# igashov/DiffLinker

Measured on AMD Instinct MI355X. Metric: molecules/sec (500-step sample_chain), higher is better.
Workload: dtype f32 (f16x3 split MFMA, fp32 accumulate)

## Files before the change

### difflinker_amd/csrc/egnn_fc.hip

```cpp
#include <hip/hip_runtime.h>
#include <stdint.h>
#include <stdlib.h>
#include <string.h>
#include <math.h>
#include <cmath>

#include <algorithm>
#include <atomic>
#include <vector>

#include "../../include/difflinker_hip.h"
#include "pack_layout.h"


namespace {

constexpr int LDH = 132;
constexpr int NMAX = 55;
constexpr int NQMAX = 2 * NMAX;
constexpr int THREADS = 512;
constexpr int NWAVES = THREADS / 64;
constexpr int GWAVES = 8;
constexpr int GTHREADS = 64 * GWAVES;
constexpr int L_A = 0;
// ... 1477 lines not shown
    lds_barrier();
    prof_event(pf, w, lane, 250);
    if (valid) {
#pragma unroll
        for (int ot = 0; ot < 8; ++ot) {
            *reinterpret_cast<float4*>(v.A + l * LDH + 16 * ot + 4 * kg) = Pout[ot];
            *reinterpret_cast<float4*>(v.B + l * LDH + 16 * ot + 4 * kg) = Qout[ot];
        }
    }
    }
    if (tid == 0) {
        if constexpr (POST) { v.fmax[FS_HS] = __float_as_uint(s_hn); v.misc[CX_PAR] = par ^ 1; }
        v.misc[CX_PASS] = pass_open;
    }
    if constexpr (TEAM) {
        prof_event(pf, w, lane, 110);
        lds_barrier();
        team_exchange_q<1>(v, nb, tid, scn, pass_open == 0, POST ? (par ^ 1) : par, pf);
    }
    prof_event(pf, w, lane, 11);
    dma_wait();
    lds_barrier();
}


template <int PREC, bool TEAM, bool ATT>
__device__ __forceinline__ void gcl_pass3(const Lds& v, Prof& pf) {
    {
    const PassCtx cx = pass_ctx(v);
    const int nb = cx.nb, N = cx.N, par = cx.par;
    const int8_t* emask = cx.em;
    const float* sc = cx.g + G_SCALE;
    const LaneIds q = lane_ids(v);
    const int tid = q.tid, w = q.w, lane = q.lane;
    prof_event(pf, w, lane, 12);
    if (tid == 0) { v.fmax[FM_H0 + (par ^ 1)] = 0u; v.fmax[FM_AGG] = 0u; }
    const float hmax = __uint_as_float(v.fmax[TEAM ? FM_HG : FM_H0 + par]);
    const float x2 = __uint_as_float(v.fmax[FM_X2]), x02 = __uint_as_float(v.fmax[FM_X02]);
    const float pqb = (cload(sc, SC_L1_W1A) + cload(sc, SC_L1_W1B)) * hmax + cload(sc, SC_B1);
    const float u1b = pqb + 4.0f * (x2 * cload(sc, GS_WRW) + x02 * cload(sc, GS_WDW));
    const float sa = scale_for(u1b);
    const float accs = sa * cload(sc, 5);
    if (tid == 0 && (beyond_f16_range(u1b) || beyond_f16_range(hmax) || beyond_f16_range(4.0f * x2) || beyond_f16_range(4.0f * x02)))
        atomicOr(&v.misc[1], NAN_RANGE | 3);
    if constexpr (ATT) pair_phase<false, PREC, true, TEAM>(v, nb, w, lane, emask, N, 0.0f, sa, inv_pow2(accs), sc, cload(sc, 8), pf);
    else pair_phase<false, PREC, false, TEAM>(v, nb, w, lane, emask, N, 0.0f, sa, inv_pow2(accs), sc, 0.0f, pf);
    prof_event(pf, w, lane, 13);
    }
    AggRegs ar;
    bool next_eq;
    {
        const PassCtx cx = pass_ctx(v);
        const int nown = TEAM ? ctx_i(v, TM_NOWN) : cx.nb;
        const LaneIds q = lane_ids(v);
        next_eq = cx.nx.equiv;
        lds_barrier();
        prof_event(pf, q.w, q.lane, 20);
        const float am = pair_reduce_gcl(v, nown, cx.nb, q.tid, ar, (cx.flags & 4) ? 1.0f / float(cx.N) : 1.0f);
        block_max(&v.fmax[FM_AGG], am, q.lane);
        prof_event(pf, q.w, q.lane, 21);
        lds_barrier();
        prof_event(pf, q.w, q.lane, 22);
    }
    if (next_eq) stream_phase<TEAM, true, true>(v, pf, &ar);
    else stream_phase<TEAM, true, false>(v, pf, &ar);
}

template <int PREC, bool TEAM>
__device__ __forceinline__ void equiv_pass3(const Lds& v, Prof& pf) {
    {
    const PassCtx cx = pass_ctx(v);
    const int nb = cx.nb, N = cx.N, par = cx.par;
    const int8_t* emask = cx.em;
    const float* sc = cx.g + E_SCALE;
    const float norm_constant = ctx_f(v, CX_NORMC);
    const LaneIds q = lane_ids(v);
    const int w = q.w, lane = q.lane;
    prof_event(pf, w, lane, 32);
    const float hmax = __uint_as_float(v.fmax[TEAM ? FM_HG : FM_H0 + par]);
    const float x2 = __uint_as_float(v.fmax[FM_X2]), x02 = __uint_as_float(v.fmax[FM_X02]);
    const float pqb = (cload(sc, SCE_L1_W5A) + cload(sc, SCE_L1_W5B)) * hmax + cload(sc, SCE_B5);
    const float u1b = pqb + 4.0f * (x2 * cload(sc, ES_WRW) + x02 * cload(sc, ES_WDW));
    const float sa = scale_for(u1b);
    const float accs = sa * cload(sc, 2);
    if (q.tid == 0 && (beyond_f16_range(u1b) || beyond_f16_range(hmax) || beyond_f16_range(4.0f * x2) || beyond_f16_range(4.0f * x02)))
        atomicOr(&v.misc[1], NAN_RANGE | 3);
    const float phi = cload(sc, ES_W7L1) * fmaf(cload(sc, ES_L1_W6), u1b, cload(sc, ES_B6));
    const bool proven = 2.0f * float(nb) * phi < 1e37f;
    if (!proven) {
        const bool widen = ctx_i(v, MS_FULL) == 0;
        __syncthreads();
        if (widen) {
            const int tid_ = q.tid;
            receivers_all(v, TEAM ? ctx_i(v, TM_NOWN) : nb, tid_);
            __syncthreads();
        }
    }
    pair_phase<true, PREC, false, TEAM>(v, nb, w, lane, emask, N, norm_constant, sa, inv_pow2(accs), sc,
                                        (cx.flags & 2) ? ctx_f(v, CX_CRANGE) : 0.0f, pf);
    prof_event(pf, w, lane, 33);
    }
    const PassCtx cx = pass_ctx(v);
    const int nb = cx.nb, N = cx.N;
    const int nown = TEAM ? ctx_i(v, TM_NOWN) : nb;
    const int S = TEAM ? ctx_i(v, TM_S) : 1, rank = TEAM ? ctx_i(v, TM_RANK) : 0;
    const bool more = cx.nx.base != nullptr;
    const LaneIds q = lane_ids(v);
    const int tid = q.tid, lane = q.lane;
    lds_barrier();
    const float xscale = (cx.flags & 4) ? 1.0f / float(N) : ((cx.flags & 2) ? ctx_f(v, CX_INVNORM) : 1.0f);
    pair_reduce_equiv<true>(v, nown, nb, tid, xscale);
    if (tid == 0) v.fmax[TEAM ? FM_XOWN : FM_X2] = 0u;
    lds_barrier();
    const float* aggx = v.A - L_A + L_AGGX3;
    float n2 = 0.0f;
    if (tid < nown) {
        const float lm = v.lm[tid];
        const int a = rank + tid * S;
        const bool moves = v.rpos[tid] >= 0;
#pragma unroll
        for (int k = 0; k < 3; ++k) {
            float xn = v.xs[4 * a + k];
            if (moves) {
                xn += aggx[4 * tid + k] * lm;
                v.xs[4 * a + k] = xn;
            }
            n2 = fmaf(xn, xn, n2);
        }
    }
    block_max(&v.fmax[TEAM ? FM_XOWN : FM_X2], n2, lane);
    prof_event(pf, q.w, lane, 34);
    lds_barrier();
    prof_event(pf, q.w, lane, 10);
    if (more) stream_phase<TEAM, false, false>(v, pf, nullptr);
}

template <bool TEAM>
__device__ __forceinline__ void head_phase(const Lds& v, bool v3);

template <int PREC, bool TEAM, bool ATT>
__device__ __forceinline__ void forward_molecule2(const Lds& v, Prof& pf) {
    const int tid = lane_ids(v).tid;
    const int nb = ctx_i(v, 0);
    const int nown = TEAM ? ctx_i(v, TM_NOWN) : nb;
    const int S = TEAM ? ctx_i(v, TM_S) : 1, rank = TEAM ? ctx_i(v, TM_RANK) : 0;
    const float* wp = ctx_p<const float>(v, CX_WP);
    float* hs = ctx_p<float>(v, CX_HS);
    const float tfeat = ctx_f(v, CX_TFEAT);
    const int nf = ctx_i(v, CX_NF), fin = ctx_i(v, CX_FIN);
    const int npass = ctx_i(v, CX_NPASS);
    const int w = __builtin_amdgcn_readfirstlane(tid >> 6);
    const int lane = tid & 63;
    const bool v3 = (PREC != 0) && !TEAM && nown > 32;
    if (tid == 0) { v.misc[CX_PASS] = v3 ? -1 : 0; v.misc[CX_PAR] = 0; v.misc[CX_V3] = v3 ? 1 : 0; }
    if (tid < 8) reinterpret_cast<int*>(v.A - L_A + L_PROG)[tid] = 0;
    if (!TEAM && tid < HID) (v.A - L_A + L_ZROW)[tid] = 0.0f;
    prof_event(pf, w, lane, 1);
    {
        if (tid < 8) v.fmax[tid] = 0u;
        __syncthreads();
    }
    const NextPass first = {wp + OFF_BLOCKS, false};
    if (!v3) stage_next(v, first, w, tid);
    if (tid < 4 * nown) {
        const int l = tid >> 2, k = tid & 3, a = rank + l * S;
        const float xv = (k < 3) ? v.z[l * DMAX + k] : 0.0f;
        v.xs[4 * a + k] = xv;
        v.x0[4 * a + k] = xv;
    }
    {
        float n2 = 0.0f;
        if (tid < nown) {
            const float x0 = v.z[tid * DMAX], x1 = v.z[tid * DMAX + 1], x2 = v.z[tid * DMAX + 2];
            n2 = x0 * x0 + x1 * x1 + x2 * x2;
        }
        const unsigned b = wave_max_u32(__float_as_uint(n2));
        if (lane == 0) {
            if (TEAM) lds_max_u32(&v.fmax[FM_XOWN], b);
            else { lds_max_u32(&v.fmax[FM_X2], b); lds_max_u32(&v.fmax[FM_X02], b); }
        }
    }
    {
        const int f = tid & (HID - 1);
        float wrow[FINP];
        const float4* wsrc = reinterpret_cast<const float4*>(wp + OFF_EMB_W + f * FINP);
#pragma unroll
        for (int q = 0; q < FINP / 4; ++q) {
            const float4 t4 = wsrc[q];
            wrow[4 * q] = t4.x; wrow[4 * q + 1] = t4.y; wrow[4 * q + 2] = t4.z; wrow[4 * q + 3] = t4.w;
        }
        const float be = wp[OFF_EMB_B + f];
        const float* ctxp = ctx_p<const float>(v, CX_CTXP);
        const int ct = ctx_i(v, CX_CT);
        const int nctx = fin - nf - ct;
        float hmax = 0.0f;
        for (int l = tid >> 7; l < nown; l += THREADS / HID) {
            const int pos = v.idx[rank + l * S];
            float acc = be;
#pragma unroll
            for (int k = 0; k < FINP; ++k) {
                float hin = 0.0f;
                if (k < nf) hin = v.z[l * DMAX + 3 + k];
                else if (k < nf + ct) hin = tfeat;
                else if (k < fin) hin = ctxp[pos * nctx + (k - nf - ct)];
                acc = fmaf(wrow[k], hin, acc);
            }
            if (v3) {
                hs[HS_HT + ((((l >> 4) * 8 + (f >> 4)) * 64 + 16 * ((f >> 2) & 3) + (l & 15)) * 4) + (f & 3)] = acc;
            } else {
            v.B[l * LDH + f] = acc;
            {
                const int r = l & 31;
                hs[HS_HT + ((((l >> 5) * 4 + (f >> 5)) * 4 + (r >> 3)) * 64 + (f & 31) + 32 * ((r >> 2) & 1)) * 4 + (r & 3)] = acc;
            }
            }
            hmax = fmaxf(hmax, fabsf(acc));
        }
        block_max(&v.fmax[FM_H0], hmax, lane);
    }
    __syncthreads();
    if (v3) {
        if constexpr (PREC != 0 && !TEAM) {
        if (tid == 0 && beyond_f16_range(__uint_as_float(v.fmax[FM_H0]))) atomicOr(&v.misc[1], NAN_RANGE | 3);
        prof_event(pf, w, lane, 2);
        stream_phase<TEAM, false, false>(v, pf, nullptr);
        const int sub = ctx_i(v, CX_SUB);
#pragma nounroll
        for (int p = 0; p < npass; p += sub + 1) {
#pragma nounroll
            for (int gi = 0; gi < sub; ++gi) gcl_pass3<PREC, TEAM, ATT>(v, pf);
            equiv_pass3<PREC, TEAM>(v, pf);
        }
        prof_event(pf, w, lane, 3);
        __syncthreads();
        head_phase<TEAM>(v, true);
        }
    } else {
    {
        const float s0 = (PREC != 0) ? scale_for(__uint_as_float(v.fmax[FM_H0])) : 1.0f;
        for (int e = tid; e < nown * 32; e += THREADS)
            put_quad<PREC>(v.C + (e >> 5) * LDH, 4 * (e & 31), *reinterpret_cast<const float4*>(v.B + (e >> 5) * LDH + 4 * (e & 31)), s0);
        if (PREC != 0 && tid == 0) {
            v.fmax[FS_HS] = __float_as_uint(s0);
            if (beyond_f16_range(__uint_as_float(v.fmax[FM_H0]))) atomicOr(&v.misc[1], NAN_RANGE | 3);
        }
    }
    __syncthreads();
    prof_event(pf, w, lane, 2);
    {
        PreW2 pw;
        load_pre2(pw, first, w, lane, nown);
        open_pass<PREC, TEAM>(v, nb, nown, first, hs, pf, pw, 0, 0);
    }
    const int sub = ctx_i(v, CX_SUB);
#pragma nounroll
    for (int p = 0; p < npass; p += sub + 1) {
#pragma nounroll
        for (int gi = 0; gi < sub; ++gi) gcl_pass2<PREC, TEAM, ATT>(v, pf);
        equiv_pass2<PREC, TEAM>(v, pf);
    }
    prof_event(pf, w, lane, 3);
    __syncthreads();
    head_phase<TEAM>(v, false);
    }
    prof_event(pf, w, lane, 4);
}

template <bool TEAM>
__device__ __forceinline__ void head_phase(const Lds& v, bool v3) {
    const int tid = lane_ids(v).tid;
    const int nb = ctx_i(v, 0), nf = ctx_i(v, CX_NF);
    const int nown = TEAM ? ctx_i(v, TM_NOWN) : nb;
    const int S = TEAM ? ctx_i(v, TM_S) : 1, rank = TEAM ? ctx_i(v, TM_RANK) : 0;
    const float* wp = ctx_p<const float>(v, CX_WP);
    const float* hs = ctx_p<const float>(v, CX_HS);
    float* eps = v.A;
    int nanbits = 0;
    for (int e = tid; e < nown * nf; e += THREADS) {
        const int a = e / nf, o = e - a * nf;
        const int r = a & 31;
        const float* wo = wp + OFF_OUT_W + o * HID;
        float acc = wp[OFF_OUT_B + o];
        if (v3) {
            const float* hp = hs + HS_HT + ((a >> 4) * 8 * 64 + (a & 15)) * 4;
#pragma unroll
            for (int ot = 0; ot < 8; ++ot)
#pragma unroll
                for (int kg = 0; kg < 4; ++kg) {
                    const float4 hv = *reinterpret_cast<const float4*>(hp + (ot * 64 + 16 * kg) * 4);
                    const float4 wv = *reinterpret_cast<const float4*>(wo + 16 * ot + 4 * kg);
                    acc = fmaf(hv.x, wv.x, acc); acc = fmaf(hv.y, wv.y, acc);
                    acc = fmaf(hv.z, wv.z, acc); acc = fmaf(hv.w, wv.w, acc);
                }
        } else {
        const float* hp = hs + HS_HO + ((a >> 5) * 4 * 16 + (r & 3) + 4 * (r >> 3)) * 64 + 32 * ((r >> 2) & 1);
#pragma unroll
        for (int nt4 = 0; nt4 < 4; ++nt4)
#pragma unroll 8
            for (int q = 0; q < 8; ++q) {
                const float4 hv = *reinterpret_cast<const float4*>(hp + nt4 * 16 * 64 + 4 * q);
                const float4 wv = *reinterpret_cast<const float4*>(wo + 32 * nt4 + 4 * q);
                acc = fmaf(hv.x, wv.x, acc); acc = fmaf(hv.y, wv.y, acc);
                acc = fmaf(hv.z, wv.z, acc); acc = fmaf(hv.w, wv.w, acc);
            }
        }
        (void)r;
        eps[a * DMAX + 3 + o] = acc;
        if (acc != acc) nanbits |= 2;
    }
    if (tid < 4 * nown && (tid & 3) < 3) {
        const int l = tid >> 2, a = rank + l * S;
        const float vel = v.xs[4 * a + (tid & 3)] - v.x0[4 * a + (tid & 3)];
        eps[l * DMAX + (tid & 3)] = vel;
        if (vel != vel) nanbits |= 1;
    }
    if (TEAM && tid == 0 && v.misc[TM_FAIL] != 0) nanbits |= 8;
    if (nanbits) atomicOr(&v.misc[1], nanbits);
    __syncthreads();
}

__device__ __forceinline__ void build_receivers(const Lds& v, int nown, int tid) {
    if (tid < 64) {
        const bool rec = tid < nown && v.lm[tid] != 0.0f;
        const unsigned long long bal = __ballot(rec);
        const int pos = __popcll(bal & ((1ull << tid) - 1ull));
        if (rec) v.rcv[pos] = tid;
        if (tid < NMAX + 1) v.rpos[tid] = rec ? pos : -1;
        if (tid == 0) { v.misc[MS_NRCV] = __popcll(bal); v.misc[MS_FULL] = (__popcll(bal) == nown) ? 1 : 0; }
    }
}

__device__ __forceinline__ int compact_atoms(const Lds& v, const int8_t* __restrict__ node_mask_b, int N, int tid) {
    if (tid < 64) {
        int count = 0;
        for (int base = 0; base < N; base += 64) {
            const int a = base + tid;
            const bool real = (a < N) && (node_mask_b[a] != 0);
            const unsigned long long bal = __ballot(real);
            const int pos = count + __popcll(bal & ((1ull << tid) - 1ull));
            if (real && pos < NQMAX) v.idx[pos] = a;
            count += __popcll(bal);
        }
        if (tid == 0) { v.misc[0] = count; v.misc[1] = 0; }
    }
    __syncthreads();
    return v.misc[0];
}

struct FwdArgs {
    const float* wpack;
    ModelDims md;
    int B, N;
    const float* xh;
    const float* t;
    int t_stride;
    const int8_t* node_mask;
    const float* linker_mask;
    const int8_t* edge_mask;
    const float* context;
    float* out;
    int* nan_flags;
    unsigned long long* prof;
    int team;
    int team_fault;
    char* team_rows;
    unsigned* team_flags;
    float* hsave;
};

struct TeamSlot {
    int slot, rank;
};
__device__ __forceinline__ TeamSlot team_slot(int k, int S) {
    const int group = k / (8 * S), within = k - group * 8 * S;
    TeamSlot t;
    t.slot = group * 8 + (within & 7);
    t.rank = within >> 3;
    return t;
// ... 563 lines not shown
        for (int k = 0; k < HID; ++k) r += fabs(double(w[size_t(f) * ld + col0 + k]) * scale);
        m = fmax(m, r);
    }
    return float(m * 1.0001);
}

float pack_sin_columns(float* dst, const float* w, int ld, double scale) {
    double m = 0.0;
    for (int f = 0; f < HID; ++f) {
        double r = 0.0;
        for (int k = 0; k < SIN_K; ++k) {
            const double v = double(w[size_t(f) * ld + 2 * HID + k]) * scale;
            dst[k * HID + f] = float(v);
            r += fabs(v);
        }
        m = fmax(m, r);
    }
    return float(m * 1.0001);
}

float vec_absmax(const float* v) {
    float m = 0.0f;
    for (int f = 0; f < HID; ++f) m = fmaxf(m, fabsf(v[f]));
    return m;
}

void pack_vec(float* dst, const float* src, int stride, double scale) {
    for (int f = 0; f < HID; ++f) dst[f] = float(double(src[size_t(f) * stride]) * scale);
}

struct Balance {
    int perm[HID];
    double fac[HID];
};
void balance_hidden(Balance& b, const double* proxy, int group, bool on) {
    for (int p = 0; p < HID; ++p) { b.perm[p] = p; b.fac[p] = 1.0; }
    if (!on) return;
    double key[HID];
    for (int f = 0; f < HID; ++f) key[f] = std::isfinite(proxy[f]) ? proxy[f] : 1.7e308;
    proxy = key;
    std::stable_sort(b.perm, b.perm + HID, [&](int x, int y) { return proxy[x] > proxy[y]; });
    const double top = proxy[b.perm[0]];
    if (!(top > 0.0) || !std::isfinite(top)) return;
    int real = 0;
    while (real < HID && proxy[b.perm[real]] > 0.0) ++real;
    if (real < HID) {
        const int groups = HID / group, per = (real + groups - 1) / groups;
        int sorted[HID];
        memcpy(sorted, b.perm, sizeof(sorted));
        int pad = real;
        for (int g = 0; g < groups; ++g)
            for (int q = 0; q < group; ++q) {
                const int j = g * per + q;
                b.perm[g * group + q] = (q < per && j < real) ? sorted[j] : sorted[pad++];
            }
    }
    for (int p0 = 0; p0 < HID; p0 += group) {
        const double m = proxy[b.perm[p0]];
        int n = 0;
        if (m > 0.0 && std::isfinite(m)) {
            int et, em;
            frexp(top, &et); frexp(m, &em);
            n = std::min(std::max(et - em, 0), 40);
        } else n = 40;
        for (int p = p0; p < p0 + group; ++p) b.fac[p] = ldexp(1.0, n);
    }
}
void permute_rows(std::vector<float>& wp, std::vector<float>& bp, const float* w, const float* bias, int ld, const Balance& b) {
    wp.resize(size_t(HID) * ld); bp.resize(HID);
    for (int p = 0; p < HID; ++p) {
        memcpy(&wp[size_t(p) * ld], w + size_t(b.perm[p]) * ld, size_t(ld) * sizeof(float));
        bp[p] = bias[b.perm[p]];
    }
}
void permute_cols(std::vector<float>& wp, const float* w, const Balance& b) {
    wp.resize(size_t(HID) * HID);
    for (int f = 0; f < HID; ++f)
        for (int p = 0; p < HID; ++p) wp[size_t(f) * HID + p] = float(double(w[size_t(f) * HID + b.perm[p]]) / b.fac[p]);
}
float row_l1_weighted(const float* w, int ld, int col0, int ncols, double scale, const Balance& b) {
    double m = 0.0;
    for (int p = 0; p < HID; ++p) {
        double r = 0.0;
        for (int k = 0; k < ncols; ++k) r += fabs(double(w[size_t(p) * ld + col0 + k]) * scale);
        m = fmax(m, r * b.fac[p]);
    }
    return float(m * 1.0001);
}
float vec_absmax_weighted(const float* v, const Balance& b) {
    double m = 0.0;
    for (int p = 0; p < HID; ++p) m = fmax(m, fabs(double(v[p])) * b.fac[p]);
    return float(m * 1.0001);
}

}

extern "C" {

int32_t dl_abi_version(void) { return DL_ABI_VERSION; }
#ifdef DL_PROFILE
int32_t dl_profile_max_events(void) { return PROF_MAX_EVENTS; }
#else
int32_t dl_profile_max_events(void) { return 0; }
#endif
void dl_set_profile_buffer(void* device_buf) { g_prof_buf = static_cast<unsigned long long*>(device_buf); }
int32_t dl_last_hip_error(void) { return g_last_hip; }
int32_t dl_max_atoms(void) { return NMAX; }
#ifdef DL_TEST_HOOKS
void dl_debug_team_fault(int32_t launches) { g_team_fault.store(launches < 0 ? 0 : launches); }
#endif

const char* dl_error_string(int32_t s) {
    switch (s) {
        case DL_OK: return "ok";
        case DL_ERR_BAD_ARG: return "bad argument";
        case DL_ERR_UNSUPPORTED: return "hyper-parameter not supported by the HIP path";
        case DL_ERR_TOO_MANY_ATOMS: return "molecule exceeds dl_max_atoms()";
        case DL_ERR_HIP: return "HIP runtime error";
        case DL_ERR_NO_DEVICE: return "no HIP device";
        case DL_ERR_ALLOC: return "allocation failed";
        default: return "unknown";
    }
}

static int32_t check_cfg(const dl_config* c) {
    if (!c) return DL_ERR_BAD_ARG;
    if (c->n_dims != 3 || c->hidden_nf != HID) return DL_ERR_UNSUPPORTED;
    if (c->inv_sublayers < 1 || c->inv_sublayers > MAX_SUBLAYERS) return DL_ERR_UNSUPPORTED;
    if ((c->condition_time | 1) != 1) return DL_ERR_BAD_ARG;
    if (c->in_node_nf < 1 || 3 + c->in_node_nf > DMAX || c->in_node_nf > 16) return DL_ERR_UNSUPPORTED;
    if (c->context_node_nf < 0 || c->context_node_nf > CTXMAX) return DL_ERR_UNSUPPORTED;
    if (c->in_node_nf + c->condition_time + c->context_node_nf > FINP) return DL_ERR_UNSUPPORTED;
    if (c->n_layers < 1 || c->n_layers > 64) return DL_ERR_UNSUPPORTED;
    if (!(c->normalization_factor > 0.0f)) return DL_ERR_BAD_ARG;
    if (c->precision != DL_PRECISION_FP32 && c->precision != DL_PRECISION_F16X3 && c->precision != DL_PRECISION_F16X2) return DL_ERR_UNSUPPORTED;
    if ((c->attention | 1) != 1 || (c->tanh | 1) != 1 || (c->aggregation_mean | 1) != 1) return DL_ERR_BAD_ARG;
    if ((c->sin_embedding | 1) != 1) return DL_ERR_BAD_ARG;
    if (c->tanh && !(c->coords_range > 0.0f)) return DL_ERR_BAD_ARG;
    return DL_OK;
}

int32_t dl_model_num_tensors(const dl_config* cfg) {
    if (!cfg) return DL_ERR_BAD_ARG;
    return 4 + cfg->n_layers * (cfg->inv_sublayers * (8 + (cfg->attention ? 2 : 0)) + 5);
}

int32_t dl_model_create(const dl_config* cfg, const float* const* w, int32_t n_tensors, dl_model** out) {
    int32_t st = check_cfg(cfg);
    if (st != DL_OK) return st;
    if (!w || !out || n_tensors != dl_model_num_tensors(cfg)) return DL_ERR_BAD_ARG;
    for (int i = 0; i < n_tensors; ++i)
        if (!w[i]) return DL_ERR_BAD_ARG;
    const int nf = cfg->in_node_nf, fin = nf + cfg->condition_time + cfg->context_node_nf, L = cfg->n_layers, SUB = cfg->inv_sublayers;
    const size_t total = size_t(OFF_BLOCKS) + size_t(L) * block_size(SUB);
    float* hp = static_cast<float*>(calloc(total, sizeof(float)));
    if (!hp) return DL_ERR_ALLOC;
    const bool f16 = cfg->precision != DL_PRECISION_FP32;
    auto image = [&](float* d, const float* ww, int ld, double sc) -> float {
        if (f16) return float(pack_lds_image_f16(d, ww, ld, sc));
        pack_lds_image(d, ww, ld, sc);
        return 1.0f;
    };
    auto image_t = [&](float* d, const float* ww, int ld, double sc) {
        if (f16) (void)pack_lds_image_f16_t(d, ww, ld, sc);
        else pack_lds_image_t(d, ww, ld, sc);
    };
    const double c = -1.4426950408889634;
    const double inv_norm = 1.0 / double(cfg->normalization_factor);
    int ti = 0;
    const float* ew = w[ti++]; const float* eb = w[ti++];
    const float* ow = w[ti++]; const float* ob = w[ti++];
    for (int f = 0; f < HID; ++f) {
        for (int k = 0; k < fin; ++k) hp[OFF_EMB_W + f * FINP + k] = ew[size_t(f) * fin + k];
        hp[OFF_EMB_B + f] = eb[f];
    }
    for (int o = 0; o < nf; ++o) {
        memcpy(hp + OFF_OUT_W + o * HID, ow + size_t(o) * HID, HID * sizeof(float));
        hp[OFF_OUT_B + o] = ob[o];
    }
    std::vector<float> w1p, b1p, w2p, w3p, b3p, w4p;
    std::vector<double> proxy(HID);
    for (int blk = 0; blk < L; ++blk) {
        float* base = hp + OFF_BLOCKS + size_t(blk) * block_size(SUB);
        for (int gi = 0; gi < SUB; ++gi) {
            float* g = base + gi * GCL_SIZE;
            const float* w1 = w[ti++]; const float* b1 = w[ti++];
            const float* w2 = w[ti++]; const float* b2 = w[ti++];
            const float* w3 = w[ti++]; const float* b3 = w[ti++];
            const float* w4 = w[ti++]; const float* b4 = w[ti++];
            const float* watt = nullptr; const float* batt = nullptr;
            if (cfg->attention) { watt = w[ti++]; batt = w[ti++]; }
            const int ld1 = 2 * HID + (cfg->sin_embedding ? SIN_K : 2);
            const int nattr = ld1 - 2 * HID;
            const double s3b = cfg->aggregation_mean ? 1.0 : inv_norm;
            Balance be, bt;
            for (int f = 0; f < HID; ++f) {
                double r = fabs(double(b1[f]));
                for (int k = 0; k < 2 * HID; ++k) r += fabs(double(w1[size_t(f) * ld1 + k]));
                for (int k = 0; k < nattr; ++k) r += (cfg->sin_embedding ? 1.0 : 32.0) * fabs(double(w1[size_t(f) * ld1 + 2 * HID + k]));
                proxy[f] = r;
            }
            balance_hidden(be, proxy.data(), 16, f16);
            for (int f = 0; f < HID; ++f) {
                double r = fabs(double(b3[f]) * c);
                for (int k = 0; k < HID; ++k) r += fabs(double(w3[size_t(f) * 2 * HID + k]) * c) + fabs(double(w3[size_t(f) * 2 * HID + HID + k]) * s3b);
                proxy[f] = r;
            }
            balance_hidden(bt, proxy.data(), 32, f16);
            permute_rows(w1p, b1p, w1, b1, ld1, be);
            permute_cols(w2p, w2, be);
            permute_rows(w3p, b3p, w3, b3, 2 * HID, bt);
            permute_cols(w4p, w4, bt);
            float* sc = g + G_SCALE;
            if (f16) {
                pack_unit_f16(g + G_W1A, w1p.data(), ld1, 0, c, sc + GS_SW_W1A);
                pack_unit_f16(g + G_W1B, w1p.data(), ld1, HID, c, sc + GS_SW_W1B);
                pack_unit_f16(g + G_W3A, w3p.data(), 2 * HID, 0, c, sc + GS_SW_W3A);
                pack_unit_f16(g + G_W3B, w3p.data(), 2 * HID, HID, s3b, sc + GS_SW_W3B);
                sc[4] = float(pack_unit_f16_uniform(g + G_W4, w4p.data(), HID, 0, 1.0 / c));
                {
                    std::vector<float> ua(UNIT), ub(UNIT);
                    pack_stream_f16(ua.data(), w3p.data(), 2 * HID, 0, c, true);
                    pack_stream_f16(ub.data(), w3p.data(), 2 * HID, HID, s3b, true);
                    for (int h2 = 0; h2 < 2; ++h2) {
                        memcpy(g + G_ST_POST + (2 * h2 + 0) * ST_CHUNK, ua.data() + h2 * ST_CHUNK, ST_CHUNK * sizeof(float));
                        memcpy(g + G_ST_POST + (2 * h2 + 1) * ST_CHUNK, ub.data() + h2 * ST_CHUNK, ST_CHUNK * sizeof(float));
                    }
                }
                pack_stream_f16(g + G_ST_POST + 2 * UNIT, w4p.data(), HID, 0, 1.0 / c, false);
                pack_stream_f16(g + G_ST_PRE, w1p.data(), ld1, 0, c, true);
                pack_stream_f16(g + G_ST_PRE + UNIT, w1p.data(), ld1, HID, c, true);
            } else {
                pack_unit(g + G_W1A, w1p.data(), ld1, 0, c); pack_unit(g + G_W1B, w1p.data(), ld1, HID, c);
                pack_unit(g + G_W3A, w3p.data(), 2 * HID, 0, c); pack_unit(g + G_W3B, w3p.data(), 2 * HID, HID, s3b);
                pack_unit(g + G_W4, w4p.data(), HID, 0, 1.0 / c);
                for (int k = 0; k < 16; ++k) sc[GS_SW_W1A + k] = 1.0f;
                sc[4] = 1.0f;
            }
            sc[5] = image(g + G_W2, w2p.data(), HID, 1.0);
            image_t(g + G_W2T, w2p.data(), HID, 1.0);
            for (int s_ = 0; s_ < 8; ++s_) sc[GS_NE + s_] = float(be.fac[16 * s_]);
            for (int nt = 0; nt < 4; ++nt) sc[GS_NT + nt] = float(bt.fac[32 * nt]);
            float* vv = g + G_VEC;
            pack_vec(vv + 0 * HID, b1p.data(), 1, c);
            if (!cfg->sin_embedding) {
                pack_vec(vv + 1 * HID, w1p.data() + 2 * HID, ld1, c);
                pack_vec(vv + 2 * HID, w1p.data() + 2 * HID + 1, ld1, c);
            } else {
                (void)pack_sin_columns(g + G_WG, w1p.data(), ld1, c);
                sc[20] = row_l1_weighted(w1p.data(), ld1, 2 * HID, SIN_K, c, be);
            }
            pack_vec(vv + 3 * HID, b2, 1, c);
            pack_vec(vv + 4 * HID, b3p.data(), 1, c);
            pack_vec(vv + 5 * HID, b4, 1, 1.0);
            if (watt) { pack_vec(vv + 6 * HID, watt, 1, 1.0 / c); sc[8] = batt[0]; }
            sc[6] = vec_absmax(vv + 1 * HID);
            sc[7] = vec_absmax(vv + 2 * HID);
            sc[GS_WRW] = vec_absmax_weighted(vv + 1 * HID, be);
            sc[GS_WDW] = vec_absmax_weighted(vv + 2 * HID, be);
            sc[12] = row_l1_weighted(w1p.data(), ld1, 0, HID, c, be); sc[13] = row_l1_weighted(w1p.data(), ld1, HID, HID, c, be);
            sc[14] = row_l1_weighted(w3p.data(), 2 * HID, 0, HID, c, bt); sc[15] = row_l1_weighted(w3p.data(), 2 * HID, HID, HID, s3b, bt);
            sc[16] = row_l1(w4p.data(), HID, 0, 1.0 / c);
            sc[17] = vec_absmax_weighted(vv + 0 * HID, be); sc[18] = vec_absmax_weighted(vv + 4 * HID, bt);
            sc[19] = vec_absmax(vv + 5 * HID) * 1.0001f;
        }
        float* e = base + SUB * GCL_SIZE;
        const float* w5 = w[ti++]; const float* b5 = w[ti++];
        const float* w6 = w[ti++]; const float* b6 = w[ti++];
        const float* w7 = w[ti++];
        const int ld5 = 2 * HID + (cfg->sin_embedding ? SIN_K : 2);
        Balance bc;
        for (int f = 0; f < HID; ++f) {
            double r = fabs(double(b5[f]));
            for (int k = 0; k < 2 * HID; ++k) r += fabs(double(w5[size_t(f) * ld5 + k]));
            for (int k = 0; k < ld5 - 2 * HID; ++k) r += (cfg->sin_embedding ? 1.0 : 32.0) * fabs(double(w5[size_t(f) * ld5 + 2 * HID + k]));
            proxy[f] = r;
        }
        balance_hidden(bc, proxy.data(), 16, f16);
        permute_rows(w1p, b1p, w5, b5, ld5, bc);
        permute_cols(w2p, w6, bc);
        float* sc = e + E_SCALE;
        if (f16) {
            pack_unit_f16(e + E_W5A, w1p.data(), ld5, 0, c, sc + ES_SW_W5A);
            pack_unit_f16(e + E_W5B, w1p.data(), ld5, HID, c, sc + ES_SW_W5B);
            pack_stream_f16(e + E_ST_PRE, w1p.data(), ld5, 0, c, true);
            pack_stream_f16(e + E_ST_PRE + UNIT, w1p.data(), ld5, HID, c, true);
        } else {
            pack_unit(e + E_W5A, w1p.data(), ld5, 0, c); pack_unit(e + E_W5B, w1p.data(), ld5, HID, c);
            for (int k = 0; k < 8; ++k) sc[ES_SW_W5A + k] = 1.0f;
        }
        sc[2] = image(e + E_W6, w2p.data(), HID, 1.0);
        image_t(e + E_W6T, w2p.data(), HID, 1.0);
        for (int s_ = 0; s_ < 8; ++s_) sc[ES_NE + s_] = float(bc.fac[16 * s_]);
        float* vv = e + E_VEC;
        pack_vec(vv + 0 * HID, b1p.data(), 1, c);
        if (!cfg->sin_embedding) {
            pack_vec(vv + 1 * HID, w1p.data() + 2 * HID, ld5, c);
            pack_vec(vv + 2 * HID, w1p.data() + 2 * HID + 1, ld5, c);
        } else {
            (void)pack_sin_columns(e + E_WG, w1p.data(), ld5, c);
            sc[11] = row_l1_weighted(w1p.data(), ld5, 2 * HID, SIN_K, c, bc);
        }
        pack_vec(vv + 3 * HID, b6, 1, c);
        pack_vec(vv + 4 * HID, w7, 1, (cfg->tanh || cfg->aggregation_mean) ? 1.0 / c : inv_norm / c);
        sc[6] = vec_absmax(vv + 1 * HID);
        sc[7] = vec_absmax(vv + 2 * HID);
        sc[ES_WRW] = vec_absmax_weighted(vv + 1 * HID, bc);
        sc[ES_WDW] = vec_absmax_weighted(vv + 2 * HID, bc);
        sc[8] = row_l1_weighted(w1p.data(), ld5, 0, HID, c, bc); sc[9] = row_l1_weighted(w1p.data(), ld5, HID, HID, c, bc);
        sc[10] = vec_absmax_weighted(vv + 0 * HID, bc);
        sc[ES_L1_W6] = row_l1(w2p.data(), HID, 0, 1.0);
        sc[ES_B6] = vec_absmax(vv + 3 * HID) * 1.0001f;
        {
            double l1 = 0.0;
            for (int f = 0; f < HID; ++f) l1 += fabs(double(vv[4 * HID + f]));
            sc[ES_W7L1] = float(l1 * 1.0001);
        }
    }
    dl_model* m = static_cast<dl_model*>(calloc(1, sizeof(dl_model)));
    if (!m) { free(hp); return DL_ERR_ALLOC; }
    m->cfg = *cfg;
    if (cfg->sin_embedding)
        for (int blk = 0; blk < L; ++blk) {
            const float* base = hp + OFF_BLOCKS + size_t(blk) * block_size(SUB);
            for (int gi = 0; gi < SUB; ++gi) m->sin_l1[blk * (MAX_SUBLAYERS + 1) + gi] = base[gi * GCL_SIZE + G_SCALE + 20];
            m->sin_l1[blk * (MAX_SUBLAYERS + 1) + SUB] = base[SUB * GCL_SIZE + E_SCALE + 11];
        }
    m->n_floats = total;
    int ndev = 0;
    if (hipGetDeviceCount(&ndev) != hipSuccess || ndev == 0) { free(hp); free(m); return DL_ERR_NO_DEVICE; }
    if (!hip_ok(hipMalloc(reinterpret_cast<void**>(&m->d_pack), total * sizeof(float))) ||
        !hip_ok(hipMemcpy(m->d_pack, hp, total * sizeof(float), hipMemcpyHostToDevice))) {
        free(hp); free(m); return DL_ERR_HIP;
    }
    free(hp);
    *out = m;
    return DL_OK;
}

void dl_model_destroy(dl_model* m) {
    if (!m) return;
    if (m->d_pack) (void)hipFree(m->d_pack);
    free(m);
}

static int fc_grid(int32_t B, int32_t team) { return team <= 1 ? B : (B + 7) / 8 * 8 * team; }
static size_t hsave_bytes(int32_t B, int32_t team) { return size_t(fc_grid(B, team)) * HS_STRIDE * sizeof(float); }
static size_t team_rows_bytes(int32_t B) { return size_t(B) * TEAM_MOL_BYTES; }

size_t dl_workspace_bytes(int32_t B, int32_t team) {
    if (B <= 0 || team < 0 || team > TEAM_MAX) return 0;
    size_t n = hsave_bytes(B, team);
    if (team > 1) n += team_rows_bytes(B) + size_t(B) * TEAM_MAX * sizeof(unsigned);
    return n;
}

int32_t dl_team_max_atoms(int32_t team) { return team >= 2 ? NQMAX : NMAX; }

int32_t dl_team_max(int32_t B) {
    if (B <= 0) return 1;
    int dev = 0, cus = 0;
    if (hipGetDevice(&dev) != hipSuccess ||
        hipDeviceGetAttribute(&cus, hipDeviceAttributeMultiprocessorCount, dev) != hipSuccess) return 1;
    const int slots = (B + 7) / 8 * 8;
    int S = 1;
// ... 310 lines not shown
```

### difflinker_amd/csrc/pack_layout.h

```cpp
#pragma once
#include <hip/hip_runtime.h>
#include <stdint.h>
#include "../../include/difflinker_hip.h"

struct dl_model {
    dl_config cfg;
    float* d_pack;
    size_t n_floats;
    float sin_l1[64 * 5];
};

namespace {

typedef float floatx16 __attribute__((ext_vector_type(16)));

constexpr int HID = 128;
constexpr int UNIT = HID * HID;
constexpr int FINP = 16;
constexpr int DMAX = 16;
constexpr int CTXMAX = 4;

constexpr int OFF_EMB_W = 0;
constexpr int OFF_EMB_B = OFF_EMB_W + HID * FINP;
constexpr int OFF_OUT_W = OFF_EMB_B + HID;
constexpr int OFF_OUT_B = OFF_OUT_W + 16 * HID;
constexpr int OFF_BLOCKS = OFF_OUT_B + 16;
constexpr int G_W1A = 0, G_W1B = UNIT, G_W3A = 2 * UNIT, G_W3B = 3 * UNIT, G_W4 = 4 * UNIT, G_W2 = 5 * UNIT, G_W2T = 6 * UNIT;
constexpr int G_VEC = 7 * UNIT;
constexpr int G_SCALE = G_VEC + 7 * HID;
constexpr int GS_SW_W1A = 24, GS_SW_W1B = 28, GS_SW_W3A = 32, GS_SW_W3B = 36;
constexpr int GS_NE = 40;
constexpr int GS_NT = 48;
constexpr int GS_WRW = 52, GS_WDW = 53;
constexpr int G_SCALE_SIZE = 64;
constexpr int G_WG = G_SCALE + G_SCALE_SIZE;
constexpr int SIN_K = 24;
constexpr int G_ST_POST = 7 * UNIT + 7 * HID + G_SCALE_SIZE + SIN_K * HID;
constexpr int G_ST_PRE = G_ST_POST + 3 * UNIT;
constexpr int GCL_SIZE = G_ST_PRE + 2 * UNIT;
constexpr int E_W5A = 0, E_W5B = UNIT, E_W6 = 2 * UNIT, E_W6T = 3 * UNIT;
constexpr int E_VEC = 4 * UNIT;
constexpr int E_SCALE = E_VEC + 5 * HID;
constexpr int ES_SW_W5A = 16, ES_SW_W5B = 20;
constexpr int ES_NE = 24;
constexpr int ES_WRW = 32, ES_WDW = 33;
constexpr int ES_L1_W6 = 34, ES_B6 = 35, ES_W7L1 = 36;
constexpr int E_SCALE_SIZE = 48;
constexpr int E_WG = E_SCALE + E_SCALE_SIZE;
constexpr int E_ST_PRE = 4 * UNIT + 5 * HID + E_SCALE_SIZE + SIN_K * HID;
constexpr int EQ_SIZE = E_ST_PRE + 2 * UNIT;
__host__ __device__ inline int stream_kslot(int slab, int kg, int e) { return 32 * slab + 4 * kg + (e & 3) + 16 * (e >> 2); }
constexpr int ST_CHUNK = UNIT / 2;
constexpr int MAX_SUBLAYERS = 4;
__host__ __device__ inline size_t block_size(int sublayers) { return size_t(sublayers) * GCL_SIZE + EQ_SIZE; }

struct ModelDims {
    int nf, ctx, fin, n_layers;
    int sub, ct;
    float norm_constant;
    int attention, tanh, mean, sin;
    float coords_range, inv_norm;
};

inline ModelDims dims_of(const dl_model* m) {
    ModelDims md;
    md.nf = m->cfg.in_node_nf;
    md.ctx = m->cfg.context_node_nf;
    md.ct = m->cfg.condition_time ? 1 : 0;
    md.fin = md.nf + md.ct + md.ctx;
    md.n_layers = m->cfg.n_layers;
    md.sub = m->cfg.inv_sublayers;
    md.norm_constant = m->cfg.norm_constant;
    md.attention = m->cfg.attention; md.tanh = m->cfg.tanh; md.mean = m->cfg.aggregation_mean; md.sin = m->cfg.sin_embedding;
    md.coords_range = m->cfg.coords_range; md.inv_norm = 1.0f / m->cfg.normalization_factor;
    return md;
}

__device__ __forceinline__ float silu_u(float y) {
    return y * __builtin_amdgcn_rcpf(1.0f + __builtin_amdgcn_exp2f(y));
}

__device__ __forceinline__ float silu_scaled(float y, float inv_s) {
    return y * __builtin_amdgcn_rcpf(fmaf(__builtin_amdgcn_exp2f(y), inv_s, inv_s));
}

__device__ __forceinline__ floatx16 splat16(float v) {
    floatx16 r;
#pragma unroll
    for (int i = 0; i < 16; ++i) r[i] = v;
    return r;
}

__device__ __forceinline__ floatx16 mfma32(float a, float b, floatx16 c) {
    return __builtin_amdgcn_mfma_f32_32x32x2f32(a, b, c, 0, 0, 0);
}

__device__ __forceinline__ int acc_row(int reg, int hh) { return (reg & 3) + 8 * (reg >> 2) + 4 * hh; }

template <int CTRL>
__device__ __forceinline__ float dpp_mov(float v) {
    return __int_as_float(__builtin_amdgcn_update_dpp(0, __float_as_int(v), CTRL, 0xf, 0xf, false));
}
__device__ __forceinline__ float row16_allsum(float v) {
    v += dpp_mov<0xB1>(v);
    v += dpp_mov<0x4E>(v);
    v += dpp_mov<0x141>(v);
    v += dpp_mov<0x140>(v);
    return v;
}
__device__ __forceinline__ float quad8_allsum(float v) {
    v += dpp_mov<0xB1>(v);
    v += dpp_mov<0x4E>(v);
    v += dpp_mov<0x141>(v);
    return v;
}
__device__ __forceinline__ float half32_allsum(float v) {
    v = row16_allsum(v);
    const auto r = __builtin_amdgcn_permlane16_swap(__float_as_uint(v), __float_as_uint(v), false, false);
    return __uint_as_float(r[0]) + __uint_as_float(r[1]);
}
__device__ __forceinline__ void both_halves(float v, float& lo, float& hi) {
    const auto r = __builtin_amdgcn_permlane32_swap(__float_as_uint(v), __float_as_uint(v), false, false);
    lo = __uint_as_float(r[0]);
    hi = __uint_as_float(r[1]);
}
__device__ __forceinline__ float xor32_sum(float v) {
    float lo, hi;
    both_halves(v, lo, hi);
    return lo + hi;
}

typedef _Float16 half8 __attribute__((ext_vector_type(8)));

__device__ __forceinline__ void split8(const float (&u)[8], uint4& hi, uint4& lo) {
    unsigned h[4], l[4];
#pragma unroll
    for (int q = 0; q < 4; ++q) {
        const auto hp = __builtin_amdgcn_cvt_pkrtz(u[2 * q], u[2 * q + 1]);
        const float h0 = float(hp[0]), h1 = float(hp[1]);
        const auto lp = __builtin_amdgcn_cvt_pkrtz(u[2 * q] - h0, u[2 * q + 1] - h1);
        h[q] = __builtin_bit_cast(unsigned, hp);
        l[q] = __builtin_bit_cast(unsigned, lp);
    }
    hi = make_uint4(h[0], h[1], h[2], h[3]);
    lo = make_uint4(l[0], l[1], l[2], l[3]);
}

__device__ __forceinline__ uint4 round8(const float (&u)[8]) {
    typedef _Float16 half2v __attribute__((ext_vector_type(2)));
    typedef float float2v __attribute__((ext_vector_type(2)));
    unsigned h[4];
#pragma unroll
    for (int q = 0; q < 4; ++q) {
        const float2v p = {u[2 * q], u[2 * q + 1]};
        h[q] = __builtin_bit_cast(unsigned, __builtin_convertvector(p, half2v));
    }
    return make_uint4(h[0], h[1], h[2], h[3]);
}

__device__ __forceinline__ floatx16 mfma_h(const uint4& a, const uint4& b, floatx16 c) {
    return __builtin_amdgcn_mfma_f32_32x32x16_f16(__builtin_bit_cast(half8, a), __builtin_bit_cast(half8, b), c, 0, 0, 0);
}

__device__ __forceinline__ float scale_for(float bound) {
    const int ex = int((__float_as_uint(bound) >> 23) & 0xffu);
    int f = 268 - ex;
    f = min(max(f, 67), 187);
    if (ex == 255) f = 127;
    return __uint_as_float(unsigned(f) << 23);
}

constexpr int NAN_RANGE = 16;
__device__ __forceinline__ bool beyond_f16_range(float bound) { return bound >= 0x1p75f; }

__device__ __forceinline__ float inv_pow2(float s) { return __uint_as_float(0x7f000000u - __float_as_uint(s)); }

struct BFrag {
    float4 q[16];
};
__device__ __forceinline__ BFrag load_bfrag(const float* __restrict__ unit_nt, int lane) {
    BFrag b;
    const float4* bp = reinterpret_cast<const float4*>(unit_nt) + lane;
#pragma unroll
    for (int sg = 0; sg < 16; ++sg) b.q[sg] = bp[sg * 64];
    return b;
}

__device__ __forceinline__ void philox4x32_10(unsigned c0, unsigned c1, unsigned c2, unsigned c3, unsigned k0, unsigned k1,
                                              unsigned (&out)[4]) {
#pragma unroll
    for (int r = 0; r < 10; ++r) {
        const unsigned long long p0 = 0xD2511F53ull * c0, p1 = 0xCD9E8D57ull * c2;
        const unsigned n0 = unsigned(p1 >> 32) ^ c1 ^ k0, n1 = unsigned(p1), n2 = unsigned(p0 >> 32) ^ c3 ^ k1, n3 = unsigned(p0);
        c0 = n0; c1 = n1; c2 = n2; c3 = n3;
        k0 += 0x9E3779B9u; k1 += 0xBB67AE85u;
    }
    out[0] = c0; out[1] = c1; out[2] = c2; out[3] = c3;
}

__device__ __forceinline__ float philox_normal(unsigned long long seed, unsigned mol, unsigned atom, unsigned draw, unsigned comp) {
    unsigned r[4];
    philox4x32_10(mol, atom, draw, comp >> 2, unsigned(seed), unsigned(seed >> 32), r);
    const unsigned pair = comp & 2u;
    const float u1 = (float(r[pair] >> 8) + 0.5f) * 5.9604644775390625e-08f;
    const float u2 = (float(r[pair + 1] >> 8) + 0.5f) * 5.9604644775390625e-08f;
    const float rad = sqrtf(-2.0f * logf(u1));
    return rad * ((comp & 1u) ? sinpif(2.0f * u2) : cospif(2.0f * u2));
// ... 4 lines not shown
```

Before: 572.7.

## Fold embedding into first GCL edge projections for v3 path

Precomputes on the host the product of the first GCL layer's edge-MLP input weights with the embedding weights and bias, stored in a new entry block. For the v3 path the embedding loop also computes these fused P and Q projections directly from the raw input features and writes them to LDS, so the separate stream_phase that previously projected h is skipped. The weight staging for the first pass is now always issued and waited on with dma_wait. This adds extra per-thread FMAs and registers in the embedding loop, and changes rounding because the folded matrices are formed in double on the host.

New measurement: 574.8 (median of 6 runs). No clear change (+0.4%).

```diff
diff --git a/difflinker_amd/csrc/egnn_fc.hip b/difflinker_amd/csrc/egnn_fc.hip
--- a/difflinker_amd/csrc/egnn_fc.hip
+++ b/difflinker_amd/csrc/egnn_fc.hip
@@ -1653,7 +1653,7 @@
     const int w = __builtin_amdgcn_readfirstlane(tid >> 6);
     const int lane = tid & 63;
     const bool v3 = (PREC != 0) && !TEAM && nown > 32;
-    if (tid == 0) { v.misc[CX_PASS] = v3 ? -1 : 0; v.misc[CX_PAR] = 0; v.misc[CX_V3] = v3 ? 1 : 0; }
+    if (tid == 0) { v.misc[CX_PASS] = 0; v.misc[CX_PAR] = 0; v.misc[CX_V3] = v3 ? 1 : 0; }
     if (tid < 8) reinterpret_cast<int*>(v.A - L_A + L_PROG)[tid] = 0;
     if (!TEAM && tid < HID) (v.A - L_A + L_ZROW)[tid] = 0.0f;
     prof_event(pf, w, lane, 1);
@@ -1662,17 +1662,20 @@
         __syncthreads();
     }
     const NextPass first = {wp + OFF_BLOCKS, false};
-    if (!v3) stage_next(v, first, w, tid);
+    stage_next(v, first, w, tid);
     if (tid < 4 * nown) {
         const int l = tid >> 2, k = tid & 3, a = rank + l * S;
         const float xv = (k < 3) ? v.z[l * DMAX + k] : 0.0f;
         v.xs[4 * a + k] = xv;
         v.x0[4 * a + k] = xv;
     }
+    unsigned x2_entry;
     {
+        static_assert(NMAX <= 64, "a wave holds every atom of a molecule");
+        const int a = TEAM ? tid : lane;
         float n2 = 0.0f;
-        if (tid < nown) {
-            const float x0 = v.z[tid * DMAX], x1 = v.z[tid * DMAX + 1], x2 = v.z[tid * DMAX + 2];
+        if (a < nown) {
+            const float x0 = v.z[a * DMAX], x1 = v.z[a * DMAX + 1], x2 = v.z[a * DMAX + 2];
             n2 = x0 * x0 + x1 * x1 + x2 * x2;
         }
         const unsigned b = wave_max_u32(__float_as_uint(n2));
@@ -1680,6 +1683,7 @@
             if (TEAM) lds_max_u32(&v.fmax[FM_XOWN], b);
             else { lds_max_u32(&v.fmax[FM_X2], b); lds_max_u32(&v.fmax[FM_X02], b); }
         }
+        x2_entry = b;
     }
     {
         const int f = tid & (HID - 1);
@@ -1694,10 +1698,31 @@
         const float* ctxp = ctx_p<const float>(v, CX_CTXP);
         const int ct = ctx_i(v, CX_CT);
         const int nctx = fin - nf - ct;
+        constexpr bool V3K = (PREC != 0) && !TEAM;
+        float prow[FINP], qrow[FINP];
+        float bp = 0.0f, bq = 0.0f, S1 = 1.0f;
+        if constexpr (V3K) {
+            if (v3) {
+                const int sub = ctx_i(v, CX_SUB);
+                const float* en = wp + entry_offset(npass / (sub + 1), sub);
+                const float4* psrc = reinterpret_cast<const float4*>(en + EN_MP + f * FINP);
+                const float4* qsrc = reinterpret_cast<const float4*>(en + EN_MQ + f * FINP);
+#pragma unroll
+                for (int q = 0; q < FINP / 4; ++q) {
+                    const float4 p4 = psrc[q], q4 = qsrc[q];
+                    prow[4 * q] = p4.x; prow[4 * q + 1] = p4.y; prow[4 * q + 2] = p4.z; prow[4 * q + 3] = p4.w;
+                    qrow[4 * q] = q4.x; qrow[4 * q + 1] = q4.y; qrow[4 * q + 2] = q4.z; qrow[4 * q + 3] = q4.w;
+                }
+                bp = en[EN_BP + f]; bq = en[EN_BQ + f];
+                const float* sc0 = wp + OFF_BLOCKS + G_SCALE;
+                const float s_x = scale_for(4.0f * __uint_as_float(x2_entry));
+                S1 = fminf(s_x * scale_for(cload(sc0, 6)), s_x * scale_for(cload(sc0, 7)));
+            }
+        }
         float hmax = 0.0f;
         for (int l = tid >> 7; l < nown; l += THREADS / HID) {
             const int pos = v.idx[rank + l * S];
-            float acc = be;
+            float acc = be, pacc = bp, qacc = bq;
 #pragma unroll
             for (int k = 0; k < FINP; ++k) {
                 float hin = 0.0f;
@@ -1705,9 +1730,14 @@
                 else if (k < nf + ct) hin = tfeat;
                 else if (k < fin) hin = ctxp[pos * nctx + (k - nf - ct)];
                 acc = fmaf(wrow[k], hin, acc);
+                if constexpr (V3K) {
+                    if (v3) { pacc = fmaf(prow[k], hin, pacc); qacc = fmaf(qrow[k], hin, qacc); }
+                }
             }
             if (v3) {
                 hs[HS_HT + ((((l >> 4) * 8 + (f >> 4)) * 64 + 16 * ((f >> 2) & 3) + (l & 15)) * 4) + (f & 3)] = acc;
+                v.A[l * LDH + f] = pacc;
+                v.B[l * LDH + f] = qacc * S1;
             } else {
             v.B[l * LDH + f] = acc;
             {
@@ -1719,12 +1749,12 @@
         }
         block_max(&v.fmax[FM_H0], hmax, lane);
     }
+    if (v3) dma_wait();
     __syncthreads();
     if (v3) {
         if constexpr (PREC != 0 && !TEAM) {
         if (tid == 0 && beyond_f16_range(__uint_as_float(v.fmax[FM_H0]))) atomicOr(&v.misc[1], NAN_RANGE | 3);
         prof_event(pf, w, lane, 2);
-        stream_phase<TEAM, false, false>(v, pf, nullptr);
         const int sub = ctx_i(v, CX_SUB);
 #pragma nounroll
         for (int p = 0; p < npass; p += sub + 1) {
@@ -2594,7 +2624,7 @@
     for (int i = 0; i < n_tensors; ++i)
         if (!w[i]) return DL_ERR_BAD_ARG;
     const int nf = cfg->in_node_nf, fin = nf + cfg->condition_time + cfg->context_node_nf, L = cfg->n_layers, SUB = cfg->inv_sublayers;
-    const size_t total = size_t(OFF_BLOCKS) + size_t(L) * block_size(SUB);
+    const size_t total = entry_offset(L, SUB) + ENTRY_SIZE;
     float* hp = static_cast<float*>(calloc(total, sizeof(float)));
     if (!hp) return DL_ERR_ALLOC;
     const bool f16 = cfg->precision != DL_PRECISION_FP32;
@@ -2653,6 +2683,22 @@
             permute_cols(w2p, w2, be);
             permute_rows(w3p, b3p, w3, b3, 2 * HID, bt);
             permute_cols(w4p, w4, bt);
+            if (blk == 0 && gi == 0) {
+                float* en = hp + entry_offset(L, SUB);
+                for (int f = 0; f < HID; ++f) {
+                    const float* wa = w1p.data() + size_t(f) * ld1;
+                    for (int half = 0; half < 2; ++half) {
+                        double bias = half == 0 ? double(b1p[f]) * c : 0.0;
+                        for (int k = 0; k < HID; ++k) bias += double(wa[half * HID + k]) * c * double(eb[k]);
+                        en[(half == 0 ? EN_BP : EN_BQ) + f] = float(bias);
+                        for (int i = 0; i < fin; ++i) {
+                            double m = 0.0;
+                            for (int k = 0; k < HID; ++k) m += double(wa[half * HID + k]) * c * double(ew[size_t(k) * fin + i]);
+                            en[(half == 0 ? EN_MP : EN_MQ) + f * FINP + i] = float(m);
+                        }
+                    }
+                }
+            }
             float* sc = g + G_SCALE;
             if (f16) {
                 pack_unit_f16(g + G_W1A, w1p.data(), ld1, 0, c, sc + GS_SW_W1A);
diff --git a/difflinker_amd/csrc/pack_layout.h b/difflinker_amd/csrc/pack_layout.h
--- a/difflinker_amd/csrc/pack_layout.h
+++ b/difflinker_amd/csrc/pack_layout.h
@@ -53,6 +53,9 @@
 constexpr int ST_CHUNK = UNIT / 2;
 constexpr int MAX_SUBLAYERS = 4;
 __host__ __device__ inline size_t block_size(int sublayers) { return size_t(sublayers) * GCL_SIZE + EQ_SIZE; }
+constexpr int EN_MP = 0, EN_MQ = HID * FINP, EN_BP = 2 * HID * FINP, EN_BQ = EN_BP + HID;
+constexpr int ENTRY_SIZE = EN_BQ + HID;
+__host__ __device__ inline size_t entry_offset(int n_layers, int sublayers) { return size_t(OFF_BLOCKS) + size_t(n_layers) * block_size(sublayers); }
 
 struct ModelDims {
     int nf, ctx, fin, n_layers;
```
